# jizongFox/Deep-Co-Training-for-Semi-Supervised-Image-Segmentation

Measured on AMD Instinct MI355X. Metric: co-train imgs/sec/node (lab+unlab), 2xUNet ACDC 256x256, higher is better.
Workload: dtype bf16; 1 GPU; cfg2: 2xUNet co-training (CE + JSD), ACDC-shaped 256x256 C=4, bs 8+8 per GPU; global_batch=8+8, parallelism=dp1, inputs=blob-structured synthetic slices (tests/helpers.py::blob_batches)

## Files before the change

### deep-co-training-for-semi-supervised-image-segmentation_amd/csrc/igemm.hip

```cpp
#include <algorithm>
#include "igemm_common.h"

extern int g_tune_lean;

namespace {


template <typename T> struct Mfma;
template <> struct Mfma<bf16_t> {
  static constexpr int KSTEP = 16;
  __device__ static __forceinline__ void run(const char* a_row, const char* b_row, int half, f32x16& acc, int kk) {
    const bf16x8 a = *reinterpret_cast<const bf16x8*>(a_row + kk * 32 + half * 16);
    const bf16x8 b = *reinterpret_cast<const bf16x8*>(b_row + kk * 32 + half * 16);
    acc = __builtin_amdgcn_mfma_f32_32x32x16_bf16(a, b, acc, 0, 0, 0);
  }
};
template <> struct Mfma<float> {
  static constexpr int KSTEP = 2;
  __device__ static __forceinline__ void run(const char* a_row, const char* b_row, int half, f32x16& acc, int kk) {
    const float a = *reinterpret_cast<const float*>(a_row + (kk * 2 + half) * 4);
    const float b = *reinterpret_cast<const float*>(b_row + (kk * 2 + half) * 4);
    acc = __builtin_amdgcn_mfma_f32_32x32x2f32(a, b, acc, 0, 0, 0);
  }
};
// ... 778 lines not shown
  }
  const int tid_e = TH == 16 ? wave * 64 + (int)__builtin_amdgcn_mbcnt_hi(~0u, __builtin_amdgcn_mbcnt_lo(~0u, 0u)) : tid;
  int* rowY = reinterpret_cast<int*>(smem + ABUFS * A_BYTES + 2 * B_BYTES - BM * 8);
  int* rowM = rowY + BM;
  if (tid_e < BM) {
    const int oy = y0 + (tid_e >> 4), ox = x0 + (tid_e & 15);
    int oy_ = -1, om_ = -1;
    if (oy < p.Ho && ox < p.Wo) {
      oy_ = (int)(img * p.ysN + oy * p.ysH + ox * p.ysW);
      om_ = (int)(img * p.msN + oy * p.msH + ox * p.msW);
    }
    rowY[tid_e] = oy_; rowM[tid_e] = om_;
  }
  {
    f32x4 bv[TR];
#pragma unroll
    for (int i = 0; i < TR; ++i) bv[i] = *reinterpret_cast<const f32x4*>(biasL + wn * WTN + i * 16 + 4 * kq);
#pragma unroll
    for (int j = 0; j < PXB; ++j) {
      const int row = (PXB * wm + j) * TW + l15;
#pragma unroll
      for (int i = 0; i < TR; ++i) {
        const int cl = wn * WTN + i * 16 + 4 * kq;
        float v[4] = {acc[i][j][0] + bv[i][0], acc[i][j][1] + bv[i][1], acc[i][j][2] + bv[i][2], acc[i][j][3] + bv[i][3]};
        if (p.relu) {
#pragma unroll
          for (int e = 0; e < 4; ++e) v[e] = relu1(v[e]);
        }
        bf16x4 o;
#pragma unroll
        for (int e = 0; e < 4; ++e) o[e] = (bf16_t)v[e];
        const int chunk = (cl >> 3) ^ (row & (CPR - 1));
        *reinterpret_cast<bf16x4*>(tile + row * (BN * 2) + chunk * 16 + (cl & 4) * 2) = o;
      }
    }
  }
  __syncthreads();
  if (p.pool_y) {
    asm volatile("" ::: "memory");
    staged_pool_out<BN, NW, TH>(p, tile, img, y0, x0, n0, tid_e);
    if (p.pool_only) return;
  }
  staged_rows_out<BM, BN, NW>(p, tile, rowY, rowM, n0, tid_e);
}
template <int BN, int NWM, int NWN, int ABUFS>
__global__ __launch_bounds__(NWM * NWN * 64) void igemm3m_kernel(IgemmParams p, int tiles_x, int tiles_y) {
  igemm3m_body<BN, NWM, NWN, ABUFS, 8>(p, tiles_x, tiles_y);
}
template <int BN, int NWM, int NWN>
__global__ __launch_bounds__(NWM * NWN * 64) __attribute__((amdgpu_waves_per_eu(4, 4))) void igemm3m_tall_kernel(IgemmParams p, int tiles_x, int tiles_y) {
  igemm3m_body<BN, NWM, NWN, 1, 16>(p, tiles_x, tiles_y);
}

template <int BN, int NWM, int NWN, bool LEAN, bool RING = false>
__global__ __launch_bounds__(NWM * NWN * 64) void igemm3p_kernel(IgemmParams p, int PR, int tiles_per_img, int chunks_per_split) {
  static_assert(!RING || LEAN, "the weight ring is a form of the lean loop");
  constexpr int NW = NWM * NWN;
  constexpr int BM = 128, APIECES = 24, A_BYTES = APIECES * 1024;
  constexpr int B_BYTES = BN * 128, BPIECES = BN / 8;
  constexpr int NPA = APIECES / NW, NPB = BPIECES / NW;
  constexpr int WTN = BN / NWN, TN = WTN / 32;
  static_assert(NWM == 4 && APIECES % NW == 0 && BPIECES % NW == 0 && TN >= 1, "tile/wave mismatch");
  extern __shared__ __attribute__((aligned(128))) char smem[];
  char* Abuf = smem;
  char* Bbuf = smem + 2 * A_BYTES;

  const int tid = threadIdx.x, lane = tid & 63;
  const int wave = __builtin_amdgcn_readfirstlane(tid >> 6);
  const int wn = wave / NWM, wm = wave % NWM;
  int bxi, byi, bzi;
  if (!xcd_remap(p, bxi, byi, bzi)) return;
  const int img = bxi / tiles_per_img, ty = bxi - img * tiles_per_img;
  const int y0 = ty * PR, n0 = byi * BN;
  const int pitch = p.Wo + 2, hrows = (PR + 2) * pitch;
  const long long Ktot = 9ll * p.Cin;
  const bf16_t* xb = reinterpret_cast<const bf16_t*>(p.x);
  const char* zero = reinterpret_cast<const char*>(g_zero_page) + (lane & 7) * 16;
  const unsigned smem_l = (unsigned)(size_t)(lptr_c)(smem);

  long long aoff[NPA];
  int aoffb[NPA];
#pragma unroll
  for (int i = 0; i < NPA; ++i) {
    const int row = (wave + i * NW) * 8 + (lane >> 3);
    aoff[i] = -1;
    if (row < hrows) {
      const int hy = row / pitch, hx = row - hy * pitch;
      const int iy = y0 - p.pad_h + hy, ix = hx - p.pad_w;
      if ((unsigned)iy < (unsigned)p.Hi && (unsigned)ix < (unsigned)p.Wi)
        aoff[i] = img * p.xsN + iy * p.xsH + ix * p.xsW + (((lane & 7) ^ ((row >> 1) & 7)) * 8);
    }
    aoffb[i] = aoff[i] >= 0 ? (int)(aoff[i] * 2) : DCT_BUF_INVALID;
  }
  __amdgpu_buffer_rsrc_t rsX, rsW;
  if constexpr (LEAN) {
    rsX = __builtin_amdgcn_make_buffer_rsrc((void*)p.x, 0, (int)p.x_bytes, 0x00020000);
    rsW = __builtin_amdgcn_make_buffer_rsrc((void*)(p.w + (long long)n0 * Ktot * 2), 0, (int)(p.w_bytes - (long long)n0 * Ktot * 2), 0x00020000);
  }
  auto stageA = [&](char* buf, int c0) {
#pragma unroll
    for (int i = 0; i < NPA; ++i) {
      const char* src = aoff[i] >= 0 ? reinterpret_cast<const char*>(xb + aoff[i] + c0) : zero;
      __builtin_amdgcn_global_load_lds((gptr_t)src, (lptr_t)(buf + (wave + i * NW) * 1024), 16, 0, 0);
    }
  };
  const bf16_t* wsrc[NPB];
  int woffb[NPB];
#pragma unroll
  for (int i = 0; i < NPB; ++i) {
    const int row = (wave + i * NW) * 8 + (lane >> 3);
    wsrc[i] = reinterpret_cast<const bf16_t*>(p.w) + (long long)(n0 + row) * Ktot + (((lane & 7) ^ ((row >> 1) & 7)) * 8);
    woffb[i] = (int)(((long long)row * Ktot + (((lane & 7) ^ ((row >> 1) & 7)) * 8)) * 2);
  }
  auto stageB = [&](char* buf, int tap, int c0) {
    const long long woff = (long long)tap * p.Cin + c0;
#pragma unroll
    for (int i = 0; i < NPB; ++i)
      __builtin_amdgcn_global_load_lds((gptr_t)(wsrc[i] + woff), (lptr_t)(buf + (wave + i * NW) * 1024), 16, 0, 0);
  };

  f32x16 acc[TN];
#pragma unroll
  for (int i = 0; i < TN; ++i)
#pragma unroll
    for (int e = 0; e < 16; ++e) acc[i][e] = 0.f;

  const int half = lane >> 5, l31 = lane & 31;
  const int mpix = wm * 32 + l31;
  int rho0;
  {
    const int pr = mpix / p.Wo, pc = mpix - pr * p.Wo;
    rho0 = pr < PR ? pr * pitch + pc : 0;
  }
  const int aswz = (l31 >> 1) & 7;

  const int nch = p.Cin / 64;
  const int cbeg = bzi * chunks_per_split, cend = min(nch, cbeg + chunks_per_split);
  if constexpr (RING) {
    static_assert(A_BYTES + 3 * B_BYTES <= 80 * 1024 && A_BYTES + 3 * B_BYTES >= BM * BN * 4 + 2 * BM * 4, "ring stages / epilogue tile against 80 KiB");
    const unsigned ldsA = smem_l + wave * 1024, ldsB = smem_l + A_BYTES + wave * 1024;
    auto stA = [&](unsigned soff) {
#pragma unroll
      for (int i = 0; i < NPA; ++i) buf_lds16(rsX, ldsA + i * NW * 1024, aoffb[i], soff);
    };
    auto stB = [&](unsigned slot_off, unsigned soff) {
#pragma unroll
      for (int i = 0; i < NPB; ++i) buf_lds16(rsW, ldsB + slot_off + i * NW * 1024, woffb[i], soff);
    };
    const unsigned cin2 = (unsigned)p.Cin * 2;
    unsigned xo = (unsigned)cbeg * 128;
    unsigned wo = xo;
    int ft = 0;
    auto next_stage = [&]() {
#ifndef DCT_V3P_FREEZE_W
      if (ft < 8) wo += cin2; else wo += 128u - 8u * cin2;
#endif
      ft = ft < 8 ? ft + 1 : 0;
    };
    const int nsteps = 9 * (cend - cbeg);
    stA(xo);
    stB(0u, wo); next_stage();
    stB((unsigned)B_BYTES, wo); next_stage();
    const unsigned Wl0 = smem_l + A_BYTES + (wn * WTN + l31) * 128 + ((half ^ aswz) * 16);
    const bool wave_live = wm * 32 < PR * p.Wo;
    unsigned rs = 0, fs = 2u * B_BYTES;
    int t = 0, tapoff = 0, scol = 0;
    bool halo_issued = false;
#pragma unroll 1
    for (int k = 0; k < nsteps; ++k) {
      if (k + 1 < nsteps && !halo_issued) asm volatile("s_waitcnt vmcnt(%0)" ::"n"(NPB) : "memory");
      else asm volatile("s_waitcnt vmcnt(0)" ::: "memory");
      __builtin_amdgcn_s_barrier();
      __builtin_amdgcn_sched_barrier(0);
      if (k + 2 < nsteps) { stB(fs, wo); next_stage(); }
      __builtin_amdgcn_sched_barrier(0);
      if (wave_live) {
      const int rho = rho0 + tapoff;
      const unsigned Wl = Wl0 + rs;
      const unsigned Xl = smem_l + rho * 128 + ((half ^ ((rho >> 1) & 7)) * 16);
      bf16x8 a[2][TN], b[2];
      auto issue = [&](int set, int kk) {
#pragma unroll
        for (int i = 0; i < TN; ++i) rd128((Wl + i * 32 * 128) ^ (kk * 32), a[set][i]);
        rd128(Xl ^ (kk * 32), b[set]);
      };
      issue(0, 0);
#pragma unroll
      for (int kk = 0; kk < 4; ++kk) {
        const int set = kk & 1;
        if (kk + 1 < 4) { issue(set ^ 1, kk + 1); lgkm_wait3<TN + 1>(); } else { lgkm_wait3<0>(); }
#pragma unroll
        for (int i = 0; i < TN; ++i) touch8(a[set][i]);
        touch8(b[set]);
        __builtin_amdgcn_sched_barrier(0);
#pragma unroll
        for (int i = 0; i < TN; ++i) acc[i] = __builtin_amdgcn_mfma_f32_32x32x16_bf16(a[set][i], b[set], acc[i], 0, 0, 0);
      }
      }
      fs = rs;
      rs = rs == 2u * B_BYTES ? 0u : rs + (unsigned)B_BYTES;
      ++t; ++scol;
      const bool w3 = scol == 3, w9 = t == 9;
      tapoff += w3 ? pitch - 2 : 1;
      scol = w3 ? 0 : scol;
      tapoff = w9 ? 0 : tapoff;
      t = w9 ? 0 : t;
      xo += w9 ? 128u : 0u;
      halo_issued = w9 && k + 1 < nsteps;
      if (halo_issued) {
        __builtin_amdgcn_sched_barrier(0);
        __builtin_amdgcn_s_barrier();
        __builtin_amdgcn_sched_barrier(0);
        stA(xo);
      }
    }
    asm volatile("s_waitcnt vmcnt(0)" ::: "memory");
    __syncthreads();
  } else if constexpr (LEAN) {
    const unsigned ldsA = smem_l + wave * 1024, ldsB = smem_l + 2 * A_BYTES + wave * 1024;
    auto stA = [&](int ab_, unsigned soff) {
#pragma unroll
      for (int i = 0; i < NPA; ++i) buf_lds16(rsX, ldsA + ab_ * A_BYTES + i * NW * 1024, aoffb[i], soff);
    };
    auto stB = [&](int bb_, unsigned soff) {
#pragma unroll
      for (int i = 0; i < NPB; ++i) buf_lds16(rsW, ldsB + bb_ * B_BYTES + i * NW * 1024, woffb[i], soff);
    };
    const unsigned cin2 = (unsigned)p.Cin * 2;
    unsigned xo = (unsigned)cbeg * 128;
    unsigned wo = xo;
    stA(0, xo);
    stB(0, wo);
    __syncthreads();
    const unsigned Wl0 = smem_l + 2 * A_BYTES + (wn * WTN + l31) * 128 + ((half ^ aswz) * 16);
    int ab = 0, bb = 0;
    const int nsteps = 9 * (cend - cbeg);
    const bool wave_live = wm * 32 < PR * p.Wo;
    int t = 0, tapoff = 0, scol = 0;
#pragma unroll 1
    for (int k = 0; k < nsteps; ++k) {
      if (k + 1 < nsteps) {
#ifndef DCT_V3P_FREEZE_W
        if (t < 8) wo += cin2; else wo += 128u - 8u * cin2;
#endif
        stB(bb ^ 1, wo);
      }
      if (t == 0 && k + 9 < nsteps) stA(ab ^ 1, xo + 128u);
      if (wave_live) {
      const int rho = rho0 + tapoff;
      const unsigned Wl = Wl0 + bb * B_BYTES;
      const unsigned Xl = smem_l + ab * A_BYTES + rho * 128 + ((half ^ ((rho >> 1) & 7)) * 16);
      bf16x8 a[2][TN], b[2];
      auto issue = [&](int set, int kk) {
#pragma unroll
        for (int i = 0; i < TN; ++i) rd128((Wl + i * 32 * 128) ^ (kk * 32), a[set][i]);
        rd128(Xl ^ (kk * 32), b[set]);
      };
      issue(0, 0);
#pragma unroll
      for (int kk = 0; kk < 4; ++kk) {
        const int set = kk & 1;
// ... 232 lines not shown

template <int BM, int BN, int WM, int WN, bool BOUNDS, bool LEAN>
static void launch_v2_k(const IgemmParams& p, dim3 grid, hipStream_t st) {
  constexpr size_t stages = 2 * (size_t)(BM + BN) * 128;
  constexpr size_t lds = stages + (stages + BN * 4 <= 80 * 1024 ? (size_t)BN * 4 : 0);
  static bool attr_set = false;
  if (!attr_set) {
    (void)hipFuncSetAttribute(reinterpret_cast<const void*>(&igemm2_kernel<BM, BN, WM, WN, BOUNDS, LEAN>),
                              hipFuncAttributeMaxDynamicSharedMemorySize, (int)lds);
    attr_set = true;
  }
  DCT_LAUNCH_FAM(DCT_FAM_IGEMM2, DCT_PROF_IGEMM, (igemm2_kernel<BM, BN, WM, WN, BOUNDS, LEAN>), grid, dim3(WM * WN * 64), lds, st, p);
}
template <int BM, int BN, int WM, int WN, bool BOUNDS>
static void launch_v2(const IgemmParams& p, dim3 grid, hipStream_t st) {
  if ((g_tune_lean & 8) && p.x_bytes < (1ll << 31) && p.w_bytes < (1ll << 31) && p.R * p.S <= 32)
    launch_v2_k<BM, BN, WM, WN, BOUNDS, true>(p, grid, st);
  else launch_v2_k<BM, BN, WM, WN, BOUNDS, false>(p, grid, st);
}

template <int BN, int NWN, int ABUFS>
static void launch_v3(const IgemmParams& p, int tiles_x, int tiles_y, int images, hipStream_t st) {
  constexpr size_t lds = ABUFS * (size_t)(23 * 1024) + 2 * (size_t)BN * 128 + (size_t)BN * 4;
  static bool attr_set = false;
  if (!attr_set) {
    (void)hipFuncSetAttribute(reinterpret_cast<const void*>(&igemm3m_kernel<BN, 4, NWN, ABUFS>),
                              hipFuncAttributeMaxDynamicSharedMemorySize, (int)lds);
    attr_set = true;
  }
  const dim3 grid((unsigned)(images * tiles_y * tiles_x), p.N / BN, 1);
  DCT_LAUNCH_FAM(DCT_FAM_IGEMM3M, DCT_PROF_IGEMM, (igemm3m_kernel<BN, 4, NWN, ABUFS>), grid, dim3(4 * NWN * 64), lds, st, p, tiles_x, tiles_y);
}

template <int BN, int NWN>
static void launch_v3_tall(const IgemmParams& p, int tiles_x, int tiles_y, int images, hipStream_t st) {
  constexpr size_t lds = (size_t)(41 * 1024) + 2 * (size_t)BN * 128 + (size_t)BN * 4;
  static bool attr_set = false;
  if (!attr_set) {
    (void)hipFuncSetAttribute(reinterpret_cast<const void*>(&igemm3m_tall_kernel<BN, 4, NWN>),
                              hipFuncAttributeMaxDynamicSharedMemorySize, (int)lds);
    attr_set = true;
  }
  const dim3 grid((unsigned)(images * tiles_y * tiles_x), p.N / BN, 1);
  DCT_LAUNCH_FAM(DCT_FAM_IGEMM3M, DCT_PROF_IGEMM, (igemm3m_tall_kernel<BN, 4, NWN>), grid, dim3(4 * NWN * 64), lds, st, p, tiles_x, tiles_y);
}

struct PlanP { int use, PR, tiles_per_img, splits, cps, ring; };
int g_tune_igemm_packed = 1;
int g_tune_igemm_packed_split = 160;
int g_tune_igemm_packed_fill = 50;
int g_tune_igemm_packed_min_slices = 4;
int g_tune_igemm_packed_splits = -1;
int g_tune_igemm_packed_ring = 1;
static PlanP make_plan_p(const dct_view* x, const dct_view* y, const dct_conv_desc* d, int dtype, int N) {
  PlanP pp = {0, 0, 0, 1, 0, 0};
  if (!g_tune_igemm_halo || !g_tune_igemm_packed || dtype != DCT_BF16 || d->R != 3 || d->S != 3 || d->stride != 1 || d->dil != 1 ||
      d->scatter2x2 || x->c % 64 || N % 128 || y->w > 126)
    return pp;
  const int Wo = y->w, Ho = y->h;
  int PR = 128 / Wo;
  const int by_lds = 192 / (Wo + 2) - 2;
  if (PR > by_lds) PR = by_lds;
  if (PR > Ho) PR = Ho;
  if (PR < 1) return pp;
  const int tiles = (Ho + PR - 1) / PR;
  if ((double)Ho * Wo / (tiles * 128.0) < g_tune_igemm_packed_fill * 0.01) return pp;
  const int nch = x->c / 64;
  const long long blocks0 = (long long)y->n * tiles * (N / 128);
  const int min_slices = g_tune_igemm_packed_min_slices;
  int splits = 1;
  if (g_tune_igemm_packed_splits >= 1) {
    splits = g_tune_igemm_packed_splits < nch ? g_tune_igemm_packed_splits : nch;
  } else if (blocks0 < g_tune_igemm_packed_split) {
    splits = (int)((g_tune_igemm_packed_split + 48 + blocks0 - 1) / blocks0);
    if (splits > nch) splits = nch;
    while (splits > 1 && nch / splits < min_slices) --splits;
  }
  if ((g_tune_igemm_packed_splits < 1 && nch / splits < min_slices) ||
      blocks0 * splits < (g_tune_igemm_packed_split < 256 ? g_tune_igemm_packed_split : 256))
    return pp;
  pp.cps = (nch + splits - 1) / splits;
  pp.splits = (nch + pp.cps - 1) / pp.cps;
  pp.use = 1; pp.PR = PR; pp.tiles_per_img = tiles;
  pp.ring = g_tune_igemm_packed_ring ? 1 : 0;
  return pp;
}
template <bool LEAN, bool RING = false>
static void launch_v3p_k(const IgemmParams& p, const PlanP& pp, dim3 grid, hipStream_t st) {
  constexpr size_t lds = RING ? (size_t)(24 * 1024) + 3 * (size_t)128 * 128 : 2 * (size_t)(24 * 1024) + 2 * (size_t)128 * 128;
  static_assert(lds <= 80 * 1024, "a second block must fit the CU's LDS");
  static bool attr_set = false;
  if (!attr_set) {
    (void)hipFuncSetAttribute(reinterpret_cast<const void*>(&igemm3p_kernel<128, 4, 2, LEAN, RING>),
                              hipFuncAttributeMaxDynamicSharedMemorySize, (int)lds);
    attr_set = true;
  }
  DCT_LAUNCH_FAM(DCT_FAM_IGEMM3P, DCT_PROF_IGEMM, (igemm3p_kernel<128, 4, 2, LEAN, RING>), grid, dim3(512), lds, st, p, pp.PR, pp.tiles_per_img, pp.cps);
}
int g_tune_igemm_xcd = 1;
static dim3 xcd_grid(IgemmParams& p, dim3 grid, bool per_tap) {
  p.xcd_total = 0; p.xcd_gx = p.xcd_gy = 1;
  const long long total = (long long)grid.x * grid.y * grid.z;
  const bool want = g_tune_igemm_xcd == 2 || (g_tune_igemm_xcd == 1 && per_tap && p.w_bytes > p.x_bytes);
  if (!want || total < 16 || total > (1 << 24)) return grid;
  p.xcd_gx = (int)grid.x; p.xcd_gy = (int)grid.y; p.xcd_total = (int)total;
  return dim3((unsigned)(((total + 7) / 8) * 8), 1, 1);
}
template <typename T>
static void fold_splits(const IgemmParams& p, int splits, hipStream_t st) {
  if (splits > 1)
    DCT_LAUNCH_FAM(DCT_FAM_FOLDS, DCT_PROF_IGEMM, (splitk_epilogue_kernel<T>), dim3(div_up((long long)p.M * (p.N / 4), 256)), dim3(256), 0, st, p, splits);
}
static int v3p_loop(const IgemmParams& p, const PlanP& pp) {
  if (!((g_tune_lean & 2) && p.x_bytes < (1ll << 31) && p.w_bytes < (1ll << 31))) return 0;
  return pp.ring ? 2 : 1;
}
static void launch_v3p(const IgemmParams& p0, const PlanP& pp, int images, hipStream_t st) {
  IgemmParams p = p0;
  const dim3 grid = xcd_grid(p, dim3((unsigned)(images * pp.tiles_per_img), p.N / 128, pp.splits), false);
  switch (v3p_loop(p, pp)) {
    case 2: launch_v3p_k<true, true>(p, pp, grid, st); break;
    case 1: launch_v3p_k<true>(p, pp, grid, st); break;
    default: launch_v3p_k<false>(p, pp, grid, st); break;
  }
  fold_splits<bf16_t>(p, pp.splits, st);
}

template <typename T>
static void launch(const IgemmParams& p0, const Plan& pl, hipStream_t st) {
  IgemmParams p = p0;
  dim3 grid(div_up(p.M, pl.bm), p.N / pl.bn, pl.splits);
  if (pl.v2) {
    grid = xcd_grid(p, grid, true);
    if (pl.bn == 128) {
      if (pl.bounds) launch_v2<128, 128, 4, 2, true>(p, grid, st); else launch_v2<128, 128, 4, 2, false>(p, grid, st);
    } else {
      if (pl.bounds) launch_v2<256, 64, 8, 1, true>(p, grid, st); else launch_v2<256, 64, 8, 1, false>(p, grid, st);
    }
  } else if (pl.bn == 128) {
    DCT_LAUNCH(DCT_PROF_IGEMM, (igemm_kernel<T, 128, 128>), grid, dim3(256), 0, st, p);
  } else {
    DCT_LAUNCH(DCT_PROF_IGEMM, (igemm_kernel<T, 64, 128>), grid, dim3(256), 0, st, p);
  }
  fold_splits<T>(p, pl.splits, st);
}

}

void dct_split_dw_db_launch(const float* partial, float* scratch, float* dw, float* db, int cout, int inner, int blocks, int accumulate, hipStream_t st);
size_t dct_split_dw_db_scratch(int cout, int inner);

void dct_relu_bits_launch(const void* y_bf16, unsigned char* bits, long long chunks, hipStream_t st) {
  DCT_LAUNCH(DCT_PROF_POINTWISE, relu_bits_kernel, dim3(div_up(chunks, 256)), dim3(256), 0, st, (const bf16_t*)y_bf16, bits, chunks);
}

enum Route { ROUTE_HALO, ROUTE_HALO_STEM, ROUTE_PACKED, ROUTE_TAP };
struct ConvPlan {
  Route route;
  Plan tap;
  PlanP packed;
  int bn, tiles_x, tiles_y; long long blocks; double cover;
  int th;
  int staged;
  int fused_pool;
  int bits_after;
  size_t workspace;
};
struct ConvPtrs { bool vec16; size_t workspace_bytes; };
static bool vec16_ok(const dct_view* v, int channels) {
  return !((uintptr_t)v->ptr & 15) && v->sw % 8 == 0 && v->sh % 8 == 0 && v->sn % 8 == 0 && channels % 8 == 0 && (long long)v->n * v->sn < (1ll << 31);
}
static bool bias16_ok(const float* bias) { return !bias || !((uintptr_t)bias & 15); }
static size_t slab_bytes(int splits, int M, int N) { return splits > 1 ? (size_t)splits * M * N * sizeof(float) : 0; }
// ... 89 lines not shown
    if (!mask || dtype != DCT_BF16 || !dense(mask) || mask->c != y->c || p.mask_channels != y->c || y->c % 8) return DCT_ERR_BAD_ARG;
    p.mask_bits = d->mask_bits;
  }
  if (d->relu_bits_out) {
    if (dtype != DCT_BF16 || !dense(y) || y->c % 8 || p.scatter || ((uintptr_t)y->ptr & 15)) return DCT_ERR_BAD_ARG;
    p.bits_out = d->relu_bits_out;
  }
  if (d->stem_x) {
    if (!d->stem_dw || !d->stem_db || ((uintptr_t)d->stem_x & 3)) return DCT_ERR_BAD_ARG;
    if (dtype != DCT_BF16 || y->c != 64 || x->c != 64 || d->R != 3 || d->S != 3 || d->stride != 1 || d->dil != 1 || p.scatter || d->accumulate ||
        d->relu || bias || !d->mask_bits || d->mask_scale != 1.f || d->pool_out || d->relu_bits_out || !g_tune_igemm_halo)
      return DCT_ERR_UNSUPPORTED;
  }
  if (d->pool_only && (!d->pool_out || d->relu_bits_out)) return DCT_ERR_BAD_ARG;
  if (d->pool_codes && !d->pool_out) return DCT_ERR_BAD_ARG;
  if (d->pool_out) {
    if (p.scatter || d->accumulate || mask || d->mask_bits || ((uintptr_t)d->pool_out & 15) || ((uintptr_t)d->pool_codes & 7) || y->c % 8) return DCT_ERR_BAD_ARG;
  }
  const ConvPtrs ptrs = {vec16_ok(y, y->c) && (!mask || vec16_ok(mask, p.mask_channels)) && bias16_ok(bias), workspace ? workspace_bytes : 0};
  ConvPlan cp;
  const int rc = plan_conv(x, y, d, dtype, &ptrs, cp);
  if (rc != DCT_OK) return rc;
  p.relu = d->relu; p.accumulate = d->accumulate;
  p.kiters = cp.tap.kiters; p.kiters_per_split = cp.tap.kiters_per_split;
  p.cin_iters = x->c / cp.tap.bk;
  p.staged = cp.staged;
  p.x_bytes = view_span(x) * esz;
  p.w_bytes = (long long)p.N * d->R * d->S * x->c * esz;
  p.xcd_gx = p.xcd_gy = 1;
  p.Hp = (y->h + 1) / 2; p.Wp = (y->w + 1) / 2;
  hipStream_t st = (hipStream_t)stream;
  switch (cp.route) {
    case ROUTE_HALO_STEM:
      p.stem_x = d->stem_x; p.stem_slab = (float*)workspace;
      launch_v3<64, 1, 1>(p, cp.tiles_x, cp.tiles_y, y->n, st);
      dct_split_dw_db_launch(p.stem_slab, p.stem_slab + cp.blocks * 640, d->stem_dw, d->stem_db, 64, 9, (int)cp.blocks, d->stem_accumulate, st);
      DCT_PLAN_NOTE("igemm3m shared-halo 8x16 patches x 64 ch: %lld blocks, stem weight gradient from the tile, y not stored", cp.blocks);
      break;
    case ROUTE_HALO:
      if (cp.fused_pool) { p.pool_y = (char*)d->pool_out; p.pool_codes = d->pool_codes; p.pool_only = d->pool_only ? 1 : 0; }
      if (cp.th == 16) {
        launch_v3_tall<128, 2>(p, cp.tiles_x, cp.tiles_y, y->n, st);
      } else if (cp.bn == 128) {
        if (x->c == 64) launch_v3<128, 2, 1>(p, cp.tiles_x, cp.tiles_y, y->n, st); else launch_v3<128, 2, 2>(p, cp.tiles_x, cp.tiles_y, y->n, st);
      } else launch_v3<64, 1, 1>(p, cp.tiles_x, cp.tiles_y, y->n, st);
      DCT_PLAN_NOTE("igemm3m shared-halo %dx16 patches x %d ch: %lld blocks, cover %.0f %%, %d K-steps%s", cp.th, cp.bn, cp.blocks, cp.cover * 100, 9 * x->c / 64,
                    p.pool_y ? (p.pool_only ? ", pooled in the epilogue, y not stored" : ", pooled in the epilogue") : "");
      break;
    case ROUTE_PACKED:
      if (cp.packed.splits > 1) p.partial = (float*)workspace;
      launch_v3p(p, cp.packed, y->n, st);
      DCT_PLAN_NOTE("igemm3p packed rows (%d rows of %d px per 128-px tile): %d x %d blocks x %d channel-slice splits%s", cp.packed.PR, p.Wo,
                    y->n * cp.packed.tiles_per_img, p.N / 128, cp.packed.splits,
                    v3p_loop(p, cp.packed) == 2 ? ", weight ring (three stages, two rounds ahead)" : "");
      break;
    case ROUTE_TAP:
      if (cp.tap.splits > 1) p.partial = (float*)workspace;
      if (dtype == DCT_BF16) launch<bf16_t>(p, cp.tap, st); else launch<float>(p, cp.tap, st);
      DCT_PLAN_NOTE("%s per-tap %d x %d tile%s: %lld tiles x %d splits, %d K-steps each%s", cp.tap.v2 ? "igemm2" : "igemm", cp.tap.bm, cp.tap.bn,
                    cp.tap.bounds ? " (bounds)" : "", cp.tap.tiles, cp.tap.splits, cp.tap.kiters_per_split, p.staged ? ", staged epilogue" : "");
      break;
  }
  if (cp.bits_after) dct_relu_bits_launch(y->ptr, p.bits_out, (long long)y->n * y->h * y->w * (y->c / 8), st);
  if (d->pool_out && !cp.fused_pool) {
    dct_view pv;
    pv.ptr = d->pool_out; pv.n = y->n; pv.h = p.Hp; pv.w = p.Wp; pv.c = y->c;
    pv.sw = y->c; pv.sh = (long long)p.Wp * y->c; pv.sn = (long long)p.Hp * p.Wp * y->c;
    const int rp = d->pool_codes ? dct_maxpool2x2_fwd_codes(y, &pv, d->pool_codes, dtype, stream) : dct_maxpool2x2_fwd(y, &pv, dtype, stream);
    if (rp != DCT_OK) return rp;
  }
  return dct_check_launch();
}


int dct_tune_set_wgrad(int knob, int value);
extern int g_enet_wgrad_max_blocks;
extern int g_enet_mfma;
extern int g_stem_dgrad_mfma;
extern int g_enet_mwgrad_waves;

extern "C" int dct_tune_set(int knob, int value) {
  switch (knob) {
    case DCT_TUNE_IGEMM_SPLIT: g_tune_igemm_split = value; return DCT_OK;
    case DCT_TUNE_IGEMM_HALO: g_tune_igemm_halo = value; return DCT_OK;
    case DCT_TUNE_IGEMM_PACKED: g_tune_igemm_packed = value; return DCT_OK;
    case DCT_TUNE_IGEMM_HALO_MIN_BLOCKS: g_tune_igemm_halo_min_blocks = value; return DCT_OK;
    case DCT_TUNE_IGEMM_HALO_COVER: g_tune_igemm_halo_cover = value; return DCT_OK;
    case DCT_DIAG_IGEMM_PACKED_MIN_SLICES: if (value < 1) return DCT_ERR_BAD_ARG; g_tune_igemm_packed_min_slices = value; return DCT_OK;
    case DCT_DIAG_IGEMM_PACKED_SPLITS: g_tune_igemm_packed_splits = value; return DCT_OK;
    case DCT_TUNE_IGEMM_PACKED_RING: if (value < 0 || value > 1) return DCT_ERR_BAD_ARG; g_tune_igemm_packed_ring = value; return DCT_OK;
    case DCT_TUNE_IGEMM_HALO_TALL: if (value < 0 || value > 2) return DCT_ERR_BAD_ARG; g_tune_igemm_halo_tall = value; return DCT_OK;
    case DCT_DIAG_IGEMM_HALO_TALL_MIN_BLOCKS: if (value < 1) return DCT_ERR_BAD_ARG; g_tune_igemm_halo_tall_min_blocks = value; return DCT_OK;
    case DCT_TUNE_IGEMM_SPLIT_TARGET: if (value < 64) return DCT_ERR_BAD_ARG; g_tune_igemm_split_target = value; return DCT_OK;
    case DCT_TUNE_ENET_MWGRAD_WAVES: if (value < 64) return DCT_ERR_BAD_ARG; g_enet_mwgrad_waves = value; return DCT_OK;
    case DCT_TUNE_ENET_MFMA: if (value < 0 || value > 3) return DCT_ERR_BAD_ARG; g_enet_mfma = value; return DCT_OK;
    case DCT_TUNE_IGEMM_PACKED_SPLIT: if (value < 1) return DCT_ERR_BAD_ARG; g_tune_igemm_packed_split = value; return DCT_OK;
    case DCT_TUNE_IGEMM_PACKED_FILL: if (value < 1 || value > 100) return DCT_ERR_BAD_ARG; g_tune_igemm_packed_fill = value; return DCT_OK;
    case DCT_TUNE_IGEMM_XCD: if (value < 0 || value > 2) return DCT_ERR_BAD_ARG; g_tune_igemm_xcd = value; return DCT_OK;
    case DCT_DIAG_SKIP_FAMILIES: g_dct_skip_families = value; return DCT_OK;
    case DCT_DIAG_IGEMM_POOL: g_tune_igemm_pool = value ? 1 : 0; return DCT_OK;
    case DCT_DIAG_STEM_DGRAD_MFMA: g_stem_dgrad_mfma = value ? 1 : 0; return DCT_OK;
    case DCT_DIAG_IGEMM_SPLIT_MAX_TILES: g_tune_igemm_split_max_tiles = value; return DCT_OK;
    case DCT_DIAG_IGEMM_SPLIT_MIN_KITERS: g_tune_igemm_split_min_kiters = value; return DCT_OK;
    case DCT_TUNE_ENET_WGRAD_BLOCKS: if (value < 1 || value > 1024) return DCT_ERR_BAD_ARG; g_enet_wgrad_max_blocks = value; return DCT_OK;
    default: return dct_tune_set_wgrad(knob, value);
  }
}
```

### deep-co-training-for-semi-supervised-image-segmentation_amd/csrc/igemm_common.h

```cpp
#pragma once
#include "dct_common.h"

namespace {

struct IgemmParams {
  const char* x; const char* w; const float* bias; const char* mask; char* y;
  const unsigned char* mask_bits;
  unsigned char* bits_out;
  float* partial;
  int M, N, Cin, R, S;
  int Ho, Wo, Hi, Wi;
  int stride, dil, pad_h, pad_w;
  long long xsN, xsH, xsW;
  long long ysN, ysH, ysW;
  long long msN, msH, msW;
  int relu, scatter, accumulate, mask_channels;
  float mask_scale;
  int kiters, kiters_per_split, cin_iters;
  int cout;
  int staged;
  long long x_bytes, w_bytes;
  char* pool_y;
  unsigned char* pool_codes;
  int Hp, Wp;
// ... 119 lines not shown
      union { unsigned char b[8]; uint2 w; } cd;
#pragma unroll
      for (int i = 0; i < 8; ++i) cd.b[i] = (unsigned char)(arg[i] | (m[i] > 0.f ? 4 : 0));
      dct_store8_stream(p.pool_codes + o, cd.w);
    }
  }
}

__device__ __forceinline__ bool xcd_remap(const IgemmParams& p, int& bx, int& by, int& bz) {
  if (p.xcd_total == 0) { bx = blockIdx.x; by = blockIdx.y; bz = blockIdx.z; return true; }
  const int L = blockIdx.x, per = (p.xcd_total + 7) >> 3;
  const int logical = (L & 7) * per + (L >> 3);
  if (logical >= p.xcd_total) return false;
  bx = logical % p.xcd_gx;
  const int rest = logical / p.xcd_gx;
  by = rest % p.xcd_gy; bz = rest / p.xcd_gy;
  return true;
}

__device__ __forceinline__ float relu1(float v) {
  float r;
  asm("v_max_f32 %0, 0, %1" : "=v"(r) : "v"(v));
  return r;
}

__device__ __attribute__((aligned(128))) const uint4 g_zero_page[8] = {};

typedef __attribute__((address_space(1))) const void* gptr_t;
typedef __attribute__((address_space(3))) void* lptr_t;
typedef __attribute__((address_space(3))) const char* lptr_c;
__device__ __forceinline__ void rd128(unsigned addr, bf16x8& dst) { asm volatile("ds_read_b128 %0, %1" : "=v"(dst) : "v"(addr)); }
template <int OFF> __device__ __forceinline__ void rd128o(unsigned addr, bf16x8& dst) {
  asm volatile("ds_read_b128 %0, %1 offset:%2" : "=v"(dst) : "v"(addr), "n"(OFF));
}
__device__ __forceinline__ void rd128o_dyn(unsigned addr, int off, bf16x8& dst) {
  asm volatile("ds_read_b128 %0, %1 offset:%2" : "=v"(dst) : "v"(addr), "i"(off));
}
template <int I, int N, int STRIDE> struct RdRows {
  __device__ static __forceinline__ void run(unsigned addr, bf16x8 (&dst)[N]) {
    rd128o<I * STRIDE>(addr, dst[I]);
    if constexpr (I + 1 < N) RdRows<I + 1, N, STRIDE>::run(addr, dst);
  }
};
template <int J, int N, int STRIDE> struct RdCols {
  __device__ static __forceinline__ void run(const unsigned (&addr)[N], unsigned flip, bf16x8 (&dst)[N]) {
    rd128o<J * STRIDE>(addr[J] ^ flip, dst[J]);
    if constexpr (J + 1 < N) RdCols<J + 1, N, STRIDE>::run(addr, flip, dst);
  }
};
__device__ __forceinline__ void buf_lds16(__amdgpu_buffer_rsrc_t r, unsigned lds, int voff, unsigned soff) {
  __builtin_amdgcn_raw_ptr_buffer_load_lds(r, (lptr_t)(size_t)lds, 16, voff, (int)soff, 0, 0);
}
#define DCT_BUF_INVALID ((int)0x80000000u)
template <int N> __device__ __forceinline__ void lgkm_wait3() { asm volatile("s_waitcnt lgkmcnt(%0)" ::"n"(N) : "memory"); }
__device__ __forceinline__ void touch8(bf16x8& r) { asm volatile("" : "+v"(r)); }

}
```

### include/dct.h

```cpp
#ifndef DCT_H_
#define DCT_H_

#include <stddef.h>
#include <stdint.h>

#ifdef __cplusplus
extern "C" {
#endif

typedef enum dct_status {
  DCT_OK = 0,
  DCT_ERR_BAD_ARG = -1,
  DCT_ERR_UNSUPPORTED = -2,
  DCT_ERR_LAUNCH = -3,
  DCT_ERR_WORKSPACE = -4
} dct_status;

typedef enum dct_dtype { DCT_F32 = 0, DCT_BF16 = 1, DCT_F16 = 2 } dct_dtype;

typedef struct dct_view {
  void* ptr;
  int32_t n, h, w, c;
  int64_t sn, sh, sw;
} dct_view;
// ... 318 lines not shown

int dct_dice_counts(const float* logits, const int64_t* gt, int B, int64_t pixels_per_image, int C,
                    int32_t* inter, int32_t* psum, int32_t* gsum, dct_stream stream);

int dct_dice_update(const int32_t* inter, const int32_t* psum, const int32_t* gsum, int B, int C, int method3d,
                    uint32_t axes_mask, float smooth, float* dice, double* acc, dct_stream stream);

size_t dct_hausdorff_workspace_bytes(int B, int H, int W, int C, int method3d);
int dct_hausdorff(const float* logits , const int64_t* gt ,
                  int B, int H, int W, int C, int method3d, float sz, float sy, float sx,
                  float* hd2 , void* workspace, size_t workspace_bytes, dct_stream stream);

size_t dct_components_workspace_bytes(int B, int H, int W, int C, int method3d);
int dct_largest_component(const float* logits , int B, int H, int W, int C, int method3d, int full,
                          uint32_t class_mask, int background,
                          float* onehot , int64_t* cls ,
                          int32_t* stats , void* workspace, size_t workspace_bytes, dct_stream stream);

int dct_confusion_counts(const float* const* logits, int S, const int64_t* gt ,
                         int B, int64_t pixels_per_image, int C, int32_t* counts , dct_stream stream);

int dct_calibration_counts(const float* const* probs, int S, const int64_t* gt , int B, int64_t pixels_per_image,
                           int C, int n_bins, uint32_t class_mask, int with_ensemble, int from_logits,
                           int64_t* bins , int64_t* scores , dct_stream stream);

int dct_temperature_sums(const float* const* logits, int S, const int64_t* gt , int B, int64_t pixels_per_image,
                         int C, uint32_t class_mask, int with_ensemble, const float* betas , int K,
                         int64_t* sums , int64_t* counted , dct_stream stream);
int dct_temperature_apply(const float* const* logits, int S, int B, int64_t pixels_per_image, int C, const float* beta ,
                          int with_ensemble, float* const* out , dct_stream stream);

enum { DCT_PROF_IGEMM = 0, DCT_PROF_WGRAD = 1, DCT_PROF_POINTWISE = 2, DCT_PROF_LOSS = 3,
       DCT_PROF_ADAM = 4, DCT_PROF_OTHER = 5, DCT_PROF_NCLASS = 6 };
int dct_prof_enable(int on);
enum { DCT_TUNE_IGEMM_SPLIT = 1,
       DCT_TUNE_WGRAD_CHUNKS = 3,
       DCT_TUNE_IGEMM_HALO = 7,
       DCT_TUNE_WGRAD_ROWS = 8,
       DCT_TUNE_WGRAD_ROWS_FILL = 9,
       DCT_TUNE_IGEMM_PACKED = 10,
       DCT_TUNE_ENET_WGRAD_BLOCKS = 12,
       DCT_TUNE_WGRAD_TARGET = 14,
       DCT_TUNE_WGRAD3_TARGET = 15,
       DCT_TUNE_IGEMM_SPLIT_TARGET = 16,
       DCT_TUNE_IGEMM_HALO_MIN_BLOCKS = 19,
       DCT_TUNE_IGEMM_HALO_COVER = 20,
       DCT_TUNE_IGEMM_PACKED_SPLIT = 23,
       DCT_TUNE_IGEMM_PACKED_FILL = 24,
       DCT_TUNE_ENET_MFMA = 26,
       DCT_TUNE_ENET_MWGRAD_WAVES = 28,
       DCT_TUNE_IGEMM_XCD = 39,
       DCT_TUNE_IGEMM_HALO_TALL = 40,
       DCT_TUNE_IGEMM_PACKED_RING = 41,
       DCT_TUNE_LEAN = 38 };
int dct_tune_set(int knob, int value);
int dct_prof_read(double* ms_per_class, int64_t* launches_per_class, int reset);
int dct_clock_probe(unsigned long long* out2, unsigned long long ref_ticks, dct_stream stream);
int dct_stamp(unsigned long long* slot, unsigned ring, dct_stream stream);

typedef struct dct_enet_bwd_in {
  const dct_view* g; const dct_view* g_mask;
  const float* mean; const float* invstd; const float* c1c2;
} dct_enet_bwd_in;
int dct_enet_conv_bwd_in(const dct_view* raw, const float* w, const dct_enet_tf* tf, const dct_enet_bwd_in* bin,
                         const dct_view* y, const dct_conv_desc* d, int transposed, int ws_out, int ws_tap, int ws_in,
                         const dct_view* resid_grad, const dct_view* resid_mask, int f32_mask, int dtype,
                         const dct_view* bn_raw, const float* bn_scale, const float* bn_shift, const float* bn_slope, int bn_act,
                         const float* bn_mean, const float* bn_invstd,
                         double* stats_partial, int stats_capacity_rows, int* stats_rows, dct_stream stream);
int dct_enet_bn_bwd_sums(const dct_view* raw, const dct_view* g, const dct_view* g_mask,
                         const float* scale, const float* shift, const float* slope, int act,
                         const float* mean, const float* invstd,
                         float* dgamma, float* dbeta, float* dslope, float* c1c2, int training,
                         int f32_mask, int dtype, void* workspace, size_t workspace_bytes, int partial_rows, dct_stream stream);
int dct_enet_bn_bwd_apply(const dct_view* raw, const dct_view* g, const dct_view* g_mask,
                          const float* scale, const float* shift, const float* slope, int act,
                          const float* mean, const float* invstd, const float* c1c2,
                          const dct_view* draw, int f32_mask, int dtype, int leaf, dct_stream stream);

int dct_group_begin(int members);
int dct_group_member(int member);
int dct_group_max(void);
int dct_group_abort(void);
int dct_group_end(dct_stream stream, int* grouped_launches, int* single_launches);
int dct_leaves_begin(void);
int dct_leaves_flush(dct_stream stream, int* launches);
int dct_leaves_end(dct_stream stream, int* launches);

#ifdef __cplusplus
}
#endif
#endif
```

Measured before the change: 5024 imgs/sec.

## Prefetch next channel-slice halo through registers in packed-row igemm weight ring

```diff
diff --git a/deep-co-training-for-semi-supervised-image-segmentation_amd/csrc/igemm.hip b/deep-co-training-for-semi-supervised-image-segmentation_amd/csrc/igemm.hip
--- a/deep-co-training-for-semi-supervised-image-segmentation_amd/csrc/igemm.hip
+++ b/deep-co-training-for-semi-supervised-image-segmentation_amd/csrc/igemm.hip
@@ -854,9 +854,10 @@
   igemm3m_body<BN, NWM, NWN, 1, 16>(p, tiles_x, tiles_y);
 }
 
-template <int BN, int NWM, int NWN, bool LEAN, bool RING = false>
+template <int BN, int NWM, int NWN, bool LEAN, bool RING = false, bool HREG = false>
 __global__ __launch_bounds__(NWM * NWN * 64) void igemm3p_kernel(IgemmParams p, int PR, int tiles_per_img, int chunks_per_split) {
   static_assert(!RING || LEAN, "the weight ring is a form of the lean loop");
+  static_assert(!HREG || RING, "the register halo is a form of the weight ring");
   constexpr int NW = NWM * NWN;
   constexpr int BM = 128, APIECES = 24, A_BYTES = APIECES * 1024;
   constexpr int B_BYTES = BN * 128, BPIECES = BN / 8;
@@ -938,7 +939,89 @@
 
   const int nch = p.Cin / 64;
   const int cbeg = bzi * chunks_per_split, cend = min(nch, cbeg + chunks_per_split);
-  if constexpr (RING) {
+  if constexpr (HREG) {
+    static_assert(A_BYTES + 3 * B_BYTES <= 80 * 1024 && A_BYTES + 3 * B_BYTES >= BM * BN * 4 + 2 * BM * 4, "ring stages / epilogue tile against 80 KiB");
+    constexpr int HT = 5;
+    const unsigned ldsA = smem_l + wave * 1024, ldsB = smem_l + A_BYTES + wave * 1024;
+    const unsigned cin2 = (unsigned)p.Cin * 2;
+    unsigned xo = (unsigned)cbeg * 128;
+    const int nsl = cend - cbeg;
+    auto stB = [&](unsigned slot_off, unsigned soff) {
+#pragma unroll
+      for (int i = 0; i < NPB; ++i) buf_lds16(rsW, ldsB + slot_off + i * NW * 1024, woffb[i], soff);
+    };
+#pragma unroll
+    for (int i = 0; i < NPA; ++i) buf_lds16(rsX, ldsA + i * NW * 1024, aoffb[i], xo);
+    stB(0u, xo);
+    stB((unsigned)B_BYTES, xo + cin2);
+    const unsigned Wl0 = smem_l + A_BYTES + (wn * WTN + l31) * 128 + ((half ^ aswz) * 16);
+    const bool wave_live = wm * 32 < PR * p.Wo;
+    unsigned Xl9[9];
+#pragma unroll
+    for (int t = 0; t < 9; ++t) {
+      const int rho = rho0 + (t / 3) * pitch + t % 3;
+      Xl9[t] = smem_l + rho * 128 + ((half ^ ((rho >> 1) & 7)) * 16);
+    }
+    u32x4 hreg[NPA];
+#pragma unroll
+    for (int i = 0; i < NPA; ++i) hreg[i] = u32x4{0u, 0u, 0u, 0u};
+#pragma unroll 1
+    for (int sl = 0; sl < nsl; ++sl) {
+      const bool more = sl + 1 < nsl;
+#pragma unroll
+      for (int t = 0; t < 9; ++t) {
+        if (t == 0) asm volatile("s_waitcnt vmcnt(%0) lgkmcnt(0)" ::"n"(NPB) : "memory");
+        else if (t == HT + 1 && more) asm volatile("s_waitcnt vmcnt(%0)" ::"n"(NPB + NPA) : "memory");
+        else if (t == 8 && !more) asm volatile("s_waitcnt vmcnt(0)" ::: "memory");
+        else asm volatile("s_waitcnt vmcnt(%0)" ::"n"(NPB) : "memory");
+        __builtin_amdgcn_s_barrier();
+        __builtin_amdgcn_sched_barrier(0);
+        if (t == HT && more) {
+#pragma unroll
+          for (int i = 0; i < NPA; ++i) {
+            if (i == 0) buf_reg16<true>(rsX, aoffb[i], xo + 128u, hreg[i]); else buf_reg16<false>(rsX, aoffb[i], xo + 128u, hreg[i]);
+          }
+          __builtin_amdgcn_sched_barrier(0);
+        }
+        if (t < 7) stB((unsigned)(((t + 2) % 3) * B_BYTES), xo + (unsigned)(t + 2) * cin2);
+        else if (more) stB((unsigned)(((t + 2) % 3) * B_BYTES), xo + 128u + (unsigned)(t - 7) * cin2);
+        __builtin_amdgcn_sched_barrier(0);
+        if (wave_live) {
+        unsigned Wl = Wl0 + (unsigned)((t % 3) * B_BYTES);
+        unsigned Xl = Xl9[t];
+        asm volatile("" : "+v"(Wl), "+v"(Xl));
+        bf16x8 a[2][TN], b[2];
+        auto issue = [&](int set, int kk) {
+#pragma unroll
+          for (int i = 0; i < TN; ++i) rd128((Wl + i * 32 * 128) ^ (kk * 32), a[set][i]);
+          rd128(Xl ^ (kk * 32), b[set]);
+        };
+        issue(0, 0);
+#pragma unroll
+        for (int kk = 0; kk < 4; ++kk) {
+          const int set = kk & 1;
+          if (kk + 1 < 4) { issue(set ^ 1, kk + 1); lgkm_wait3<TN + 1>(); } else { lgkm_wait3<0>(); }
+#pragma unroll
+          for (int i = 0; i < TN; ++i) touch8(a[set][i]);
+          touch8(b[set]);
+          __builtin_amdgcn_sched_barrier(0);
+#pragma unroll
+          for (int i = 0; i < TN; ++i) acc[i] = __builtin_amdgcn_mfma_f32_32x32x16_bf16(a[set][i], b[set], acc[i], 0, 0, 0);
+        }
+        }
+        __builtin_amdgcn_sched_barrier(0);
+      }
+      xo += 128u;
+      if (more) {
+        __builtin_amdgcn_s_barrier();
+        __builtin_amdgcn_sched_barrier(0);
+#pragma unroll
+        for (int i = 0; i < NPA; ++i) wr128o_dyn(ldsA + lane * 16, i * NW * 1024, hreg[i]);
+      }
+    }
+    asm volatile("s_waitcnt vmcnt(0)" ::: "memory");
+    __syncthreads();
+  } else if constexpr (RING) {
     static_assert(A_BYTES + 3 * B_BYTES <= 80 * 1024 && A_BYTES + 3 * B_BYTES >= BM * BN * 4 + 2 * BM * 4, "ring stages / epilogue tile against 80 KiB");
     const unsigned ldsA = smem_l + wave * 1024, ldsB = smem_l + A_BYTES + wave * 1024;
     auto stA = [&](unsigned soff) {
@@ -1008,7 +1091,11 @@
       tapoff = w9 ? 0 : tapoff;
       t = w9 ? 0 : t;
       xo += w9 ? 128u : 0u;
+#ifdef DCT_V3P_NO_RESTAGE
+      halo_issued = false;
+#else
       halo_issued = w9 && k + 1 < nsteps;
+#endif
       if (halo_issued) {
         __builtin_amdgcn_sched_barrier(0);
         __builtin_amdgcn_s_barrier();
@@ -1347,6 +1434,7 @@
 int g_tune_igemm_packed_min_slices = 4;
 int g_tune_igemm_packed_splits = -1;
 int g_tune_igemm_packed_ring = 1;
+int g_tune_igemm_packed_halo_regs = 1;
 static PlanP make_plan_p(const dct_view* x, const dct_view* y, const dct_conv_desc* d, int dtype, int N) {
   PlanP pp = {0, 0, 0, 1, 0, 0};
   if (!g_tune_igemm_halo || !g_tune_igemm_packed || dtype != DCT_BF16 || d->R != 3 || d->S != 3 || d->stride != 1 || d->dil != 1 ||
@@ -1377,20 +1465,20 @@
   pp.cps = (nch + splits - 1) / splits;
   pp.splits = (nch + pp.cps - 1) / pp.cps;
   pp.use = 1; pp.PR = PR; pp.tiles_per_img = tiles;
-  pp.ring = g_tune_igemm_packed_ring ? 1 : 0;
+  pp.ring = g_tune_igemm_packed_ring ? (g_tune_igemm_packed_halo_regs ? 2 : 1) : 0;
   return pp;
 }
-template <bool LEAN, bool RING = false>
+template <bool LEAN, bool RING = false, bool HREG = false>
 static void launch_v3p_k(const IgemmParams& p, const PlanP& pp, dim3 grid, hipStream_t st) {
   constexpr size_t lds = RING ? (size_t)(24 * 1024) + 3 * (size_t)128 * 128 : 2 * (size_t)(24 * 1024) + 2 * (size_t)128 * 128;
   static_assert(lds <= 80 * 1024, "a second block must fit the CU's LDS");
   static bool attr_set = false;
   if (!attr_set) {
-    (void)hipFuncSetAttribute(reinterpret_cast<const void*>(&igemm3p_kernel<128, 4, 2, LEAN, RING>),
+    (void)hipFuncSetAttribute(reinterpret_cast<const void*>(&igemm3p_kernel<128, 4, 2, LEAN, RING, HREG>),
                               hipFuncAttributeMaxDynamicSharedMemorySize, (int)lds);
     attr_set = true;
   }
-  DCT_LAUNCH_FAM(DCT_FAM_IGEMM3P, DCT_PROF_IGEMM, (igemm3p_kernel<128, 4, 2, LEAN, RING>), grid, dim3(512), lds, st, p, pp.PR, pp.tiles_per_img, pp.cps);
+  DCT_LAUNCH_FAM(DCT_FAM_IGEMM3P, DCT_PROF_IGEMM, (igemm3p_kernel<128, 4, 2, LEAN, RING, HREG>), grid, dim3(512), lds, st, p, pp.PR, pp.tiles_per_img, pp.cps);
 }
 int g_tune_igemm_xcd = 1;
 static dim3 xcd_grid(IgemmParams& p, dim3 grid, bool per_tap) {
@@ -1408,12 +1496,13 @@
 }
 static int v3p_loop(const IgemmParams& p, const PlanP& pp) {
   if (!((g_tune_lean & 2) && p.x_bytes < (1ll << 31) && p.w_bytes < (1ll << 31))) return 0;
-  return pp.ring ? 2 : 1;
+  return pp.ring ? 1 + pp.ring : 1;
 }
 static void launch_v3p(const IgemmParams& p0, const PlanP& pp, int images, hipStream_t st) {
   IgemmParams p = p0;
   const dim3 grid = xcd_grid(p, dim3((unsigned)(images * pp.tiles_per_img), p.N / 128, pp.splits), false);
   switch (v3p_loop(p, pp)) {
+    case 3: launch_v3p_k<true, true, true>(p, pp, grid, st); break;
     case 2: launch_v3p_k<true, true>(p, pp, grid, st); break;
     case 1: launch_v3p_k<true>(p, pp, grid, st); break;
     default: launch_v3p_k<false>(p, pp, grid, st); break;
@@ -1609,7 +1698,9 @@
       launch_v3p(p, cp.packed, y->n, st);
       DCT_PLAN_NOTE("igemm3p packed rows (%d rows of %d px per 128-px tile): %d x %d blocks x %d channel-slice splits%s", cp.packed.PR, p.Wo,
                     y->n * cp.packed.tiles_per_img, p.N / 128, cp.packed.splits,
-                    v3p_loop(p, cp.packed) == 2 ? ", weight ring (three stages, two rounds ahead)" : "");
+                    v3p_loop(p, cp.packed) == 3   ? ", weight ring (three stages, two rounds ahead), next halo through registers"
+                    : v3p_loop(p, cp.packed) == 2 ? ", weight ring (three stages, two rounds ahead)"
+                                                  : "");
       break;
     case ROUTE_TAP:
       if (cp.tap.splits > 1) p.partial = (float*)workspace;
@@ -1646,6 +1737,7 @@
     case DCT_DIAG_IGEMM_PACKED_MIN_SLICES: if (value < 1) return DCT_ERR_BAD_ARG; g_tune_igemm_packed_min_slices = value; return DCT_OK;
     case DCT_DIAG_IGEMM_PACKED_SPLITS: g_tune_igemm_packed_splits = value; return DCT_OK;
     case DCT_TUNE_IGEMM_PACKED_RING: if (value < 0 || value > 1) return DCT_ERR_BAD_ARG; g_tune_igemm_packed_ring = value; return DCT_OK;
+    case DCT_TUNE_IGEMM_PACKED_HALO_REGS: if (value < 0 || value > 1) return DCT_ERR_BAD_ARG; g_tune_igemm_packed_halo_regs = value; return DCT_OK;
     case DCT_TUNE_IGEMM_HALO_TALL: if (value < 0 || value > 2) return DCT_ERR_BAD_ARG; g_tune_igemm_halo_tall = value; return DCT_OK;
     case DCT_DIAG_IGEMM_HALO_TALL_MIN_BLOCKS: if (value < 1) return DCT_ERR_BAD_ARG; g_tune_igemm_halo_tall_min_blocks = value; return DCT_OK;
     case DCT_TUNE_IGEMM_SPLIT_TARGET: if (value < 64) return DCT_ERR_BAD_ARG; g_tune_igemm_split_target = value; return DCT_OK;
diff --git a/deep-co-training-for-semi-supervised-image-segmentation_amd/csrc/igemm_common.h b/deep-co-training-for-semi-supervised-image-segmentation_amd/csrc/igemm_common.h
--- a/deep-co-training-for-semi-supervised-image-segmentation_amd/csrc/igemm_common.h
+++ b/deep-co-training-for-semi-supervised-image-segmentation_amd/csrc/igemm_common.h
@@ -195,6 +195,14 @@
   __builtin_amdgcn_raw_ptr_buffer_load_lds(r, (lptr_t)(size_t)lds, 16, voff, (int)soff, 0, 0);
 }
 #define DCT_BUF_INVALID ((int)0x80000000u)
+typedef unsigned u32x4 __attribute__((ext_vector_type(4)));
+template <bool FIRST> __device__ __forceinline__ void buf_reg16(__amdgpu_buffer_rsrc_t r, int voff, unsigned soff, u32x4& dst) {
+  if constexpr (FIRST) asm volatile("s_nop 4\n\tbuffer_load_dwordx4 %0, %1, %2, %3 offen" : "=&v"(dst) : "v"(voff), "s"(r), "s"(soff) : "memory");
+  else asm volatile("buffer_load_dwordx4 %0, %1, %2, %3 offen" : "=&v"(dst) : "v"(voff), "s"(r), "s"(soff) : "memory");
+}
+__device__ __forceinline__ void wr128o_dyn(unsigned addr, int off, const u32x4& src) {
+  asm volatile("ds_write_b128 %0, %1 offset:%2" ::"v"(addr), "v"(src), "i"(off) : "memory");
+}
 template <int N> __device__ __forceinline__ void lgkm_wait3() { asm volatile("s_waitcnt lgkmcnt(%0)" ::"n"(N) : "memory"); }
 __device__ __forceinline__ void touch8(bf16x8& r) { asm volatile("" : "+v"(r)); }
 
diff --git a/include/dct.h b/include/dct.h
--- a/include/dct.h
+++ b/include/dct.h
@@ -394,6 +394,7 @@
        DCT_TUNE_IGEMM_XCD = 39,
        DCT_TUNE_IGEMM_HALO_TALL = 40,
        DCT_TUNE_IGEMM_PACKED_RING = 41,
+       DCT_TUNE_IGEMM_PACKED_HALO_REGS = 42,
        DCT_TUNE_LEAN = 38 };
 int dct_tune_set(int knob, int value);
 int dct_prof_read(double* ms_per_class, int64_t* launches_per_class, int reset);
```

Measured after the change: 5047 imgs/sec, median of 6. About the same (+0.5%).
